# austin-hoover/ment-flow

Hardware: AMD Instinct MI355X
Metric: particle-samples/sec per MENT-Flow train step (6D, 100 proj) (higher is better)
Workload: dtype f32; 1 GPU; c4: rec_nd_1d gaussian_mixture d=6, 100 linear 1-D projections x 64 bins, NSF 5x[3x64] K=20; global_batch=2097152, per_gpu_batch=2097152, parallelism=dp1 (particle batch sharded; 2 all-reduces/step), step=zero_grad + MENTFlow.loss + backward + AdamW.step

## Files before the change

mentflow_amd/csrc/flow.hip:

```cpp
#include "flow_launch.h"
#include <stdlib.h>

namespace mf {

static int flow_check(int d, int L, int64_t n) {
    if (d < 1 || d > FLOW_DMAX) return fail("flow kernels support 1 <= d <= %d (got %d)", FLOW_DMAX, d);
    if (L < 1) return fail("hidden_layers must be >= 1");
    if (n < 0) return fail("negative particle count");
    return 0;
}

static int flow_grid(int64_t n, int waves = FLOW_WAVES) {
    const int64_t ntiles = (n + 31) / 32;
    int64_t g = (ntiles + waves - 1) / waves;
    if (g > NUM_CU) g = NUM_CU;
    if (g < 1) g = 1;
    return (int)g;
}

static int no_rqs_instance(int bins, int hidden_layers) {
    return fail("no RQS kernel instance for bins=%d hidden_layers=%d (built: 2 <= bins <= 21, hidden_layers in {1,2,3,4})", bins,
                hidden_layers);
}
static int no_affine_instance(int hidden_layers) {
    return fail("no affine kernel instance for hidden_layers=%d (built: 1 .. 4)", hidden_layers);
}

}

using namespace mf;

extern "C" int64_t mf_flow_image_floats(int d, int hidden_layers) { return image_layout(d, hidden_layers, d).total; }

static int g_bwd_variant = -1;
static bool bwd_fused_wanted() {
    static const int env_default = [] { const char* e = getenv("MENTFLOW_BWD_FUSED"); return (e && atoi(e) == 0) ? 0 : 1; }();
    return (g_bwd_variant < 0 ? env_default : g_bwd_variant) != 0;
}
extern "C" int mf_flow_set_bwd_variant(int variant) {
    if (variant < -1 || variant > 1) return fail("mf_flow_set_bwd_variant: -1 (default), 0 (two-kernel) or 1 (fused)");
    g_bwd_variant = variant;
    return 0;
}

static bool rqs_bwd_fused(int64_t n, int d, int hidden_layers, const int32_t* order, const Sparsity& sp, size_t* smem) {
    if (!bwd_fused_wanted() || order == nullptr || d > FB_DMAX) return false;
    (void)n;
    size_t fl = image_layout(d, hidden_layers, d).offW3;
    for (int i = 0; i < d; ++i) fl += (size_t)WS * (2 * ((sp.kend3[i] + 3) & ~3));
    fl += (size_t)d * HID + HID;
    fl = (fl + 3) & ~(size_t)3;
    *smem = sizeof(float) * (fl + 8 * (size_t)FB_TILE);
    return *smem <= 160 * 1024;
}

extern "C" int64_t mf_flow_bwd_scratch_floats(int64_t n, int d, int hidden_layers, const int32_t* order) {
    if (order != nullptr && d >= 1 && d <= FLOW_DMAX) {
        size_t smem;
        if (rqs_bwd_fused(n, d, hidden_layers, order, make_sparsity(d, order, d), &smem)) return 0;
    }
    const int64_t npad = ((n + 31) / 32) * 32;
    return (2 * (int64_t)hidden_layers + d) * npad * 64;
}

extern "C" int mf_flow_rqs_deriv_slot(int bins) {
    if (bins == 20 || bins == 8) return bins;
    return (bins >= 2 && bins <= RQS_KMAX) ? RQS_KMAX : -1;
}

extern "C" int mf_flow_rqs_act_level(int d, int hidden_layers, int bins, const int32_t* order) {
    if (order == nullptr || d < 1 || d > FLOW_DMAX || !rqs_saved_instance(bins, hidden_layers)) return 0;
    size_t smem;
    return rqs_bwd_fused(1, d, hidden_layers, order, make_sparsity(d, order, d), &smem) ? 2 : 0;
}
extern "C" int64_t mf_flow_rqs_act_floats(int64_t n, int d, int hidden_layers, int bins, int level) {
    if (n <= 0 || d < 1 || hidden_layers < 1 || level < 1 || level > 2) return 0;
    const int phif = bins == 20 ? phi_floats<20>() : (bins == 8 ? phi_floats<8>() : phi_floats<RQS_ANY>());
    return ((n + 31) / 32) * (int64_t)act_tile_floats(hidden_layers, level, d - 1, phif);
}

static int rqs_layer_fwd_impl(const float* image, int d, int hidden_layers, int bins, const int32_t* order, const float* x,
                              int64_t n, float* y, const float* logp_in, float* logp_out, int init_logp, float* act, int level,
                              void* stream);

extern "C" int mf_flow_rqs_layer_fwd(const float* image, int d, int hidden_layers, int bins, const int32_t* order,
                                      const float* x, int64_t n, float* y, const float* logp_in, float* logp_out,
                                      int init_logp, void* stream) {
    return rqs_layer_fwd_impl(image, d, hidden_layers, bins, order, x, n, y, logp_in, logp_out, init_logp, nullptr, 0, stream);
}

extern "C" int mf_flow_rqs_layer_fwd_save(const float* image, int d, int hidden_layers, int bins, const int32_t* order,
                                           const float* x, int64_t n, float* y, const float* logp_in, float* logp_out,
                                           int init_logp, float* act, int64_t act_floats, int level, void* stream) {
    if (level < 1 || level > 2) return fail("mf_flow_rqs_layer_fwd_save: level must be 1 or 2 (got %d)", level);
    if (level > mf_flow_rqs_act_level(d, hidden_layers, bins, order))
        return fail("no backward kernel consumes saved activations for d=%d hidden_layers=%d bins=%d (mf_flow_rqs_act_level)", d,
                    hidden_layers, bins);
    if (n > 0 && (act == nullptr || act_floats < mf_flow_rqs_act_floats(n, d, hidden_layers, bins, level)))
        return fail("act buffer too small: %lld floats, need %lld (mf_flow_rqs_act_floats)", (long long)act_floats,
                    (long long)mf_flow_rqs_act_floats(n, d, hidden_layers, bins, level));
    return rqs_layer_fwd_impl(image, d, hidden_layers, bins, order, x, n, y, logp_in, logp_out, init_logp, act, level, stream);
}

static int rqs_layer_fwd_impl(const float* image, int d, int hidden_layers, int bins, const int32_t* order, const float* x,
                              int64_t n, float* y, const float* logp_in, float* logp_out, int init_logp, float* act, int level,
                              void* stream) {
    if (flow_check(d, hidden_layers, n)) return 1;
    if (n == 0) return 0;
    const Sparsity sp = make_sparsity(d, order, d);
    const size_t smem = sizeof(float) * (size_t)image_layout(d, hidden_layers, d).total;
    const int64_t nt = (n + 31) / 32;
    const int fwd_block = nt <= 4 * NUM_CU ? 256 : (nt <= 8 * NUM_CU ? 512 : 1024);
    ProfScope prof(PK_FLOW_FWD, stream);
    if (launch_rqs_fwd(bins, hidden_layers, fwd_block, flow_grid(n, fwd_block / 64), smem, stream, image, d, x, n, y, logp_in,
                       logp_out, init_logp, sp, act, level))
        return no_rqs_instance(bins, hidden_layers);
    return check_launch("mf_flow_rqs_layer_fwd");
}

static int fused_grid(int64_t n) {
    const int64_t ngroups = ((n + 31) / 32 + 3) / 4;
    int64_t cap = NUM_CU;
#ifdef MF_EMU
    if (const char* e = getenv("MENTFLOW_EMU_FUSED_GRID")) cap = atoi(e) > 0 ? atoi(e) : cap;
#endif
    return (int)(ngroups > cap ? cap : (ngroups < 1 ? 1 : ngroups));
}
static int outer_accum_grid(int64_t n) {
    const int64_t ntiles = (n + 31) / 32;
    int64_t G = (ntiles + 7) / 8;
    if (G > 2 * NUM_CU) G = 2 * NUM_CU;
    if (G < 1) G = 1;
    return (int)G;
}

extern "C" int mf_flow_bwd_slab_rows(int64_t n, int d, int hidden_layers, const int32_t* order) {
    if (n <= 0) return 0;
    if (order != nullptr && d >= 1 && d <= FLOW_DMAX) {
        size_t smem;
        if (rqs_bwd_fused(n, d, hidden_layers, order, make_sparsity(d, order, d), &smem)) return fused_grid(n);
    }
    return outer_accum_grid(n);
}

extern "C" int mf_flow_rqs_layer_bwd_saved(const float* image, int d, int hidden_layers, int bins, const int32_t* order,
                                            const float* x, int64_t n, const float* gy, const float* glogp, float* gx,
                                            float* gslab, int slab_rows, int accumulate, const float* act, int64_t act_floats,
                                            int level, void* stream) {
    if (flow_check(d, hidden_layers, n)) return 1;
    if (n == 0) return 0;
    if (level < 1 || level > 2) return fail("mf_flow_rqs_layer_bwd_saved: level must be 1 or 2 (got %d)", level);
    if (level > mf_flow_rqs_act_level(d, hidden_layers, bins, order))
        return fail("no backward kernel consumes saved activations for d=%d hidden_layers=%d bins=%d (mf_flow_rqs_act_level)", d,
                    hidden_layers, bins);
    if (act == nullptr || act_floats < mf_flow_rqs_act_floats(n, d, hidden_layers, bins, level)) return fail("act buffer too small");
    const Sparsity sp = make_sparsity(d, order, d);
    size_t smem_f = 0;
    if (!rqs_bwd_fused(n, d, hidden_layers, order, sp, &smem_f)) return fail("the saved-activation backward is the fused kernel");
    if (slab_rows != fused_grid(n)) return fail("gslab has %d rows, this call writes %d (mf_flow_bwd_slab_rows)", slab_rows, fused_grid(n));
    ProfScope prof(PK_FLOW_BWD, stream);
    const int rc = level == 1 ? launch_rqs_bwd_fused_s1(bins, hidden_layers, fused_grid(n), smem_f, stream, image, d, x, n, gy, glogp,
                                                        gx, gslab, accumulate, sp, act)
                              : launch_rqs_bwd_fused_s2(bins, hidden_layers, fused_grid(n), smem_f, stream, image, d, x, n, gy, glogp,
// ... 173 lines not shown
```

mentflow_amd/csrc/flow_kernels.inc:

```
#include "common.h"
#include <stdlib.h>

namespace mf {

constexpr int HID = 64;
constexpr int WS = HID + 1;
constexpr int FLOW_BLOCK = 512;
constexpr int FLOW_WAVES = FLOW_BLOCK / WAVE;
constexpr int FLOW_DMAX = 7;
constexpr float RQS_BOUND = 5.0f;
constexpr float LOG_SLOPE_INV = 1.0f / 6.907755278982137f;

__device__ __forceinline__ constexpr int rowmap(int r, int hh) { return (r & 3) + 8 * (r >> 2) + 4 * hh; }

struct ImageLayout {
    int S0, offW0, offB0, offWh, offW3, offB3, total;
};
__host__ __device__ inline ImageLayout image_layout(int d, int L, int nblk) {
    ImageLayout g;
    g.S0 = d | 1;
    g.offW0 = 0;
    g.offB0 = HID * g.S0;
    g.offWh = g.offB0 + HID;
    g.offW3 = g.offWh + (L - 1) * (HID * WS + HID);
    g.offB3 = g.offW3 + nblk * HID * WS;
    g.total = g.offB3 + nblk * HID;
    return g;
}

typedef float f32x16_t __attribute__((ext_vector_type(16)));

struct Sparsity {
    int kend_h[2];
    int kbeg_ht[2];
    int kend3[FLOW_DMAX + 1];
    int rt1[FLOW_DMAX + 1];
};

static Sparsity make_sparsity(int d, const int32_t* order, int nblk) {
    Sparsity sp;
    sp.kend_h[0] = sp.kend_h[1] = 32;
    sp.kbeg_ht[0] = sp.kbeg_ht[1] = 0;
    for (int i = 0; i <= FLOW_DMAX; ++i) { sp.kend3[i] = 32; sp.rt1[i] = 1; }
    if (order == nullptr || d < 2) return sp;
    int cum[FLOW_DMAX + 2];
    for (int c = 0; c <= d; ++c) {
        int cnt = 0;
        for (int u = 0; u < HID; ++u) cnt += (1 + u % (d - 1)) <= c;
        cum[c] = cnt;
    }
    auto class_of = [&](int j) { int c = 1; while (cum[c] <= j) ++c; return c; };
    for (int rt = 0; rt < 2; ++rt) {
        sp.kend_h[rt] = (cum[class_of(32 * rt + 31)] + 1) / 2;
        sp.kbeg_ht[rt] = cum[class_of(32 * rt) - 1] / 2;
    }
    if (nblk == d) {
        for (int i = 0; i < d; ++i) {
            sp.kend3[i] = (cum[order[i]] + 1) / 2;
            sp.rt1[i] = cum[order[i]] > 32;
        }
    } else {
        sp.kend3[0] = 32;
        sp.rt1[0] = 1;
    }
    return sp;
}

#define MF_NO_HOIST() asm volatile("" ::: "memory")

__device__ __forceinline__ f32x16_t mfma(float a, float b, f32x16_t c) {
    return __builtin_amdgcn_mfma_f32_32x32x2f32(a, b, c, 0, 0, 0);
}

template <int BLOCK = FLOW_BLOCK>
__device__ __forceinline__ void stage_image(float* lds, const float* __restrict__ image, int total) {
    for (int i = threadIdx.x * 4; i < total; i += BLOCK * 4)
        *reinterpret_cast<float4*>(lds + i) = *reinterpret_cast<const float4*>(image + i);
    __syncthreads();
}

__device__ __forceinline__ f32x16_t bias_tile(const float* b, int rt, int hh) {
    f32x16_t acc;
#pragma unroll
    for (int r = 0; r < 16; ++r) acc[r] = b[32 * rt + rowmap(r, hh)];
    return acc;
}

__device__ __forceinline__ constexpr int kcol(int s) { return 32 * (s >> 4) + rowmap(s & 15, 0); }

__device__ __forceinline__ void linear64s(const float* W, int stride, const float* b, const f32x16_t (&in)[2],
                                          f32x16_t (&out)[2], int col, int hh, int kend0, int kend1) {
#pragma unroll
    for (int rt = 0; rt < 2; ++rt) {
        f32x16_t acc = bias_tile(b, rt, hh);
        const float* wrow = W + (32 * rt + col) * stride + 4 * hh;
        const int kend = rt ? kend1 : kend0;
#pragma unroll
        for (int s4 = 0; s4 < 32; s4 += 4) {
            if (s4 < kend) {
                float a[4];
#pragma unroll
                for (int j = 0; j < 4; ++j) a[j] = wrow[kcol(s4 + j)];
#pragma unroll
                for (int j = 0; j < 4; ++j) acc = mfma(a[j], in[(s4 + j) >> 4][(s4 + j) & 15], acc);
            }
        }
        out[rt] = acc;
    }
}
__device__ __forceinline__ void linear64(const float* W, const float* b, const f32x16_t (&in)[2], f32x16_t (&out)[2],
                                         int col, int hh, int kend0, int kend1) {
    linear64s(W, WS, b, in, out, col, hh, kend0, kend1);
}

__device__ __forceinline__ void linear64_t(const float* W, const f32x16_t (&in)[2], f32x16_t (&out)[2], int col, int hh,
                                           int kbeg0, int kbeg1) {
#pragma unroll
    for (int rt = 0; rt < 2; ++rt) {
        f32x16_t acc = out[rt];
        const float* wcol = W + 4 * hh * WS + 32 * rt + col;
        const int kbeg = rt ? kbeg1 : kbeg0;
#pragma unroll
        for (int s4 = 0; s4 < 32; s4 += 4) {
            if (s4 + 4 > kbeg) {
                float a[4];
#pragma unroll
                for (int j = 0; j < 4; ++j) a[j] = wcol[kcol(s4 + j) * WS];
#pragma unroll
                for (int j = 0; j < 4; ++j) acc = mfma(a[j], in[(s4 + j) >> 4][(s4 + j) & 15], acc);
            }
        }
// ... 77 lines not shown
__device__ __forceinline__ void half_pair(int v, int hh, int& lo, int& hi) {
#ifdef MF_EMU
    const int o = __shfl_xor(v, 32);
    lo = hh ? o : v;
    hi = hh ? v : o;
#else
    (void)hh;
    const auto r = __builtin_amdgcn_permlane32_swap((unsigned)v, (unsigned)v, false, false);
    lo = (int)r[0];
    hi = (int)r[1];
#endif
}

__device__ __forceinline__ unsigned cvt_u32_sat(float f) {
#ifdef MF_EMU
    return !(f > 0.0f) ? 0u : (f >= 4294967296.0f ? 0xffffffffu : (unsigned)f);
#else
    unsigned r;
    asm("v_cvt_u32_f32_e32 %0, %1" : "=v"(r) : "v"(f));
    return r;
#endif
}

template <int N, typename T>
__device__ __forceinline__ void select_pair(const T (&t)[N + 1], int idx, T& lo, T& hi) {
    constexpr int M = (N + 1) / 2;
    T a[M][3];
#pragma unroll
    for (int j = 0; j < M; ++j) {
        a[j][0] = t[2 * j];
        a[j][1] = t[2 * j + 1 <= N ? 2 * j + 1 : N];
        a[j][2] = t[2 * j + 2 <= N ? 2 * j + 2 : N];
    }
    const int j2 = idx >> 1;
#pragma unroll
    for (int b = 0; (1 << b) < M; ++b) {
        const bool bit = ((j2 >> b) & 1) != 0;
#pragma unroll
        for (int j = 0; j + (1 << b) < M; j += 2 << b)
#pragma unroll
            for (int c = 0; c < 3; ++c) a[j][c] = bit ? a[j + (1 << b)][c] : a[j][c];
    }
    const bool odd = (idx & 1) != 0;
    lo = odd ? a[0][1] : a[0][0];
    hi = odd ? a[0][2] : a[0][1];
}

constexpr int RQS_ANY = -1;
constexpr int RQS_KMAX = 21;
#define MF_PHASE(name) ((void)0)
struct NoSink {
    __device__ __forceinline__ void operator()(int, float) const {}
};
template <int K, int MODE, class Sink = NoSink>
__device__ __forceinline__ void rqs_apply(const float (&v)[32], float x, int hh, float& y_out, float& ladj_out,
                                          float gy, float gl, float (&g)[32], float& gx_out, int kbins = 0,
                                          const Sink& sink = Sink()) {
    constexpr int KM = K > 0 ? K : RQS_KMAX;
    constexpr int KD0M = KM / 2;
    const int kb = K > 0 ? K : kbins;
    const int KD0 = kb / 2;
    const int KD1 = kb - 1 - KD0;
    constexpr float A2 = 2.0f * LOG_SLOPE_INV;
    constexpr float A1 = LOG_SLOPE_INV;
    constexpr float FIX = 2147483648.0f;
    static_assert(KM + KD0M <= 32, "spline does not fit the 32 slots of a lane half");
#define MF_BIN_ON(m) (K > 0 || (m) < kb)

    MF_PHASE("softclip_exp");
    float p[KM], pq[MODE == 1 ? KM : 1];
    float sum = 0.0f;
#pragma unroll
    for (int m = 0; m < KM; ++m) {
        const float ia = fast_rcp(fmaf(fabsf(v[m]), A2 / LOG2E, 1.0f / LOG2E));
        p[m] = MF_BIN_ON(m) ? __builtin_amdgcn_exp2f(v[m] * ia) : 0.0f;
        if (MODE == 1) pq[m] = p[m] * (ia * ia);
        sum += p[m];
    }
    MF_PHASE("prefix_search");
    const float inv = fast_rcp(sum);
    unsigned cj[KM + 1];
    cj[0] = 0u;
    const float xc = fmaf(x, 0.5f / RQS_BOUND, 0.5f);
    const unsigned xq = cvt_u32_sat(xc * FIX);
    const float fscale = inv * FIX;
    unsigned c = 0u;
    int cnt = (-RQS_BOUND < x) ? 1 : 0;
#pragma unroll
    for (int j = 0; j < KM; ++j) {
        c += cvt_u32_sat(fmaf(p[j], fscale, 0.5f));
        cj[j + 1] = c;
        cnt += (MF_BIN_ON(j) && c < xq) ? 1 : 0;
    }
    MF_PHASE("select_knots");
    {
        int lo, hi;
        half_pair(cnt, hh, lo, hi);
        cnt = (MODE == 2) ? hi : lo;
    }
    const int k = cnt - 1;
    const bool inrange = (cnt >= 1) && (cnt <= kb);
    unsigned qk, qk1;
    select_pair<KM>(cj, min(max(k, 0), kb - 1), qk, qk1);
    const float ck = (float)qk * (1.0f / FIX), ck1 = (float)qk1 * (1.0f / FIX);
    const float kn0 = RQS_BOUND * (2.0f * ck - 1.0f);
    const float kn1 = RQS_BOUND * (2.0f * ck1 - 1.0f);
    float x0, x1, y0, y1;
    half_pair(kn0, hh, x0, y0);
    half_pair(kn1, hh, x1, y1);
    const int base = hh ? KD0 : 0;
    const int nown = hh ? KD1 : KD0;
    float r0, r1;
    {
        float G[KD0M + 4];
        G[0] = G[1] = G[KD0M + 2] = G[KD0M + 3] = 0.0f;
#pragma unroll
        for (int j = 0; j < KD0M; ++j) G[2 + j] = (j < nown) ? v[KM + j] : 0.0f;
        select_pair<KD0M + 3>(G, min(max(k - base + 1, 0), KD0M + 2), r0, r1);
    }
    {
        float a, b;
        half_pair(r0, hh, a, b);
        r0 = a + b;
        half_pair(r1, hh, a, b);
        r1 = a + b;
    }
    const float d0 = fast_exp(soft_clip(r0, A1));
    const float d1 = fast_exp(soft_clip(r1, A1));

    MF_PHASE("rational_log");
    const float w = x1 - x0;
    const float iw = fast_rcp(w);
    const float hgt = y1 - y0;
    const float s = hgt * iw;
    if (MODE == 2) {
        const float yb = x - y0;
        const float bet = d0 + d1 - 2.0f * s;
        const float qa = hgt * (s - d0) + yb * bet;
        const float qb = hgt * d0 - yb * bet;
        const float qc = -s * yb;
        const float zi = 2.0f * qc / (-qb - sqrtf(qb * qb - 4.0f * qa * qc));
        y_out = inrange ? fmaf(zi, w, x0) : x;
        ladj_out = 0.0f;
        return;
    }
    const float z = (x - x0) * iw;
    const float omz = 1.0f - z;
    const float z1 = z * omz;
    const float beta = d0 + d1 - 2.0f * s;
    const float num = s * z * z + d0 * z1;
    const float den = fmaf(beta, z1, s);
    const float iden = fast_rcp(den);
    const float R = num * iden;
    const float Q = 2.0f * s * z1 + d0 * omz * omz + d1 * z * z;
    const float jac = s * s * Q * iden * iden;
    y_out = inrange ? fmaf(hgt, R, y0) : x;
    ladj_out = inrange ? __builtin_amdgcn_logf(jac) * 0.6931471805599453f : 0.0f;

    MF_PHASE("adjoint_scalar");
    if (MODE == 1) {
        const float tz = 1.0f - 2.0f * z;
        const float num_z = 2.0f * s * z + d0 * tz;
        const float den_z = beta * tz;
        const float R_z = (num_z - R * den_z) * iden;
        const float den_s = 1.0f - 2.0f * z1;
        const float R_s = (z * z - R * den_s) * iden;
        const float R_d0 = z1 * (1.0f - R) * iden;
        const float R_d1 = -R * z1 * iden;
        const float iQ = fast_rcp(Q);
        const float Q_z = 2.0f * s * tz - 2.0f * d0 * omz + 2.0f * d1 * z;
        const float l_z = Q_z * iQ - 2.0f * den_z * iden;
        const float l_s = 2.0f * fast_rcp(s) + 2.0f * z1 * iQ - 2.0f * den_s * iden;
        const float l_d0 = omz * omz * iQ - 2.0f * z1 * iden;
        const float l_d1 = z * z * iQ - 2.0f * z1 * iden;
        const float gyh = gy * hgt;
        const float Gz = gyh * R_z + gl * l_z;
        const float Gs = gyh * R_s + gl * l_s;
        const float Gd0 = gyh * R_d0 + gl * l_d0;
        const float Gd1 = gyh * R_d1 + gl * l_d1;
        const float Gh = gy * R;
        gx_out = inrange ? Gz * iw : gy;
        const float gx0 = (Gz * (z - 1.0f) + Gs * s) * iw;
        const float gx1 = -(Gz * z + Gs * s) * iw;
        const float gy0 = gy - Gh - Gs * iw;
        const float gy1 = Gh + Gs * iw;
        const float gcA = inrange ? 2.0f * RQS_BOUND * (hh ? gy0 : gx0) : 0.0f;
        const float gcB = inrange ? 2.0f * RQS_BOUND * (hh ? gy1 : gx1) : 0.0f;
        const float dot = gcA * ck + gcB * ck1;
        MF_PHASE("adjoint_logits");
        const float nrm = inv * (1.0f / (LOG2E * LOG2E));
        const float t_gt = (0.0f - dot) * nrm, d_eq = gcB * nrm, d_lt = gcA * nrm;
        const float kf = (float)k;
        float u_prev = __builtin_amdgcn_fmed3f(kf + 1.0f, 0.0f, 1.0f);
#pragma unroll
        for (int m = 0; m < KM; ++m) {
            const float u = __builtin_amdgcn_fmed3f(kf - (float)m, 0.0f, 1.0f);
            g[m] = pq[m] * fmaf(u, d_lt, fmaf(u_prev, d_eq, t_gt));
            sink(m, g[m]);
            u_prev = u;
        }
        MF_PHASE("adjoint_derivs");
        const float gr0 = inrange ? Gd0 * d0 * soft_clip_grad(r0, A1) : 0.0f;
        const float gr1 = inrange ? Gd1 * d1 * soft_clip_grad(r1, A1) : 0.0f;
#pragma unroll
        for (int j = 0; j < 32 - KM; ++j) {
            const bool own = j < nown;
            float t = 0.0f;
            t = (own && (k - 1 == base + j)) ? gr0 : t;
            t = (own && (k == base + j)) ? t + gr1 : t;
            g[KM + j] = t;
            sink(KM + j, t);
        }
    }
    MF_PHASE("end");
}
#undef MF_BIN_ON

__device__ __forceinline__ void block_linear(const float* W, const float* b, const f32x16_t (&in)[2], float (&v)[32],
                                             int col, int hh, int kend) {
    f32x16_t phi[2];
    linear64(W, b, in, phi, col, hh, kend, kend);
#pragma unroll
    for (int m = 0; m < 32; ++m) v[m] = phi[m >> 4][m & 15];
}

__device__ __forceinline__ float base_log_prob(const float* xp, int d) {
    float q = 0.0f;
    for (int j = 0; j < d; ++j) q = fmaf(xp[j], xp[j], q);
    return -0.5f * q - 0.9189385332046727f * (float)d;
}

constexpr int ACT_BLOCK = 2048;
template <int K>
__host__ __device__ constexpr int phi_slots() { return K > 0 ? ((K + K / 2 + 1) & ~1) : 32; }
template <int K>
__host__ __device__ constexpr int phi_floats() { return 64 * phi_slots<K>(); }
__host__ __device__ inline int act_tile_floats(int L, int level, int nphi, int phif) {
    return level <= 0 ? 0 : (L - 1) * ACT_BLOCK + (level >= 2 ? nphi * phif : 0);
}

typedef float act_f4 __attribute__((ext_vector_type(4)));
typedef float act_f2 __attribute__((ext_vector_type(2)));
#ifdef MF_EMU
#define MF_ACT_ST(p, v) (*(p) = (v))
#define MF_ACT_LD(p) (*(p))
#else
#define MF_ACT_ST(p, v) __builtin_nontemporal_store((v), (p))
#define MF_ACT_LD(p) __builtin_nontemporal_load(p)
#endif
__device__ __forceinline__ void act_store(float* __restrict__ blk, int lane, const f32x16_t (&a)[2]) {
    act_f4* q = reinterpret_cast<act_f4*>(blk) + lane;
#pragma unroll
    for (int rt = 0; rt < 2; ++rt)
#pragma unroll
        for (int g4 = 0; g4 < 4; ++g4) {
            const act_f4 t = {a[rt][4 * g4], a[rt][4 * g4 + 1], a[rt][4 * g4 + 2], a[rt][4 * g4 + 3]};
            MF_ACT_ST(q + (4 * rt + g4) * 64, t);
        }
}
__device__ __forceinline__ void act_load(const float* __restrict__ blk, int lane, f32x16_t (&a)[2]) {
    const act_f4* q = reinterpret_cast<const act_f4*>(blk) + lane;
#pragma unroll
    for (int rt = 0; rt < 2; ++rt)
#pragma unroll
        for (int g4 = 0; g4 < 4; ++g4) {
            const act_f4 t = MF_ACT_LD(q + (4 * rt + g4) * 64);
            a[rt][4 * g4] = t.x;
            a[rt][4 * g4 + 1] = t.y;
            a[rt][4 * g4 + 2] = t.z;
            a[rt][4 * g4 + 3] = t.w;
        }
}
template <int K>
__device__ __forceinline__ void phi_store(float* __restrict__ blk, int lane, const float (&v)[32]) {
    constexpr int NS = phi_slots<K>(), NQ = NS / 4;
    act_f4* q = reinterpret_cast<act_f4*>(blk) + lane;
#pragma unroll
    for (int g4 = 0; g4 < NQ; ++g4) {
        const act_f4 t = {v[4 * g4], v[4 * g4 + 1], v[4 * g4 + 2], v[4 * g4 + 3]};
        MF_ACT_ST(q + g4 * 64, t);
    }
    if constexpr (NS % 4 != 0) {
        const act_f2 t = {v[4 * NQ], v[4 * NQ + 1]};
        MF_ACT_ST(reinterpret_cast<act_f2*>(blk + 256 * NQ) + lane, t);
    }
}
template <int K>
__device__ __forceinline__ void phi_load(const float* __restrict__ blk, int lane, float (&v)[32]) {
    constexpr int NS = phi_slots<K>(), NQ = NS / 4;
    const act_f4* q = reinterpret_cast<const act_f4*>(blk) + lane;
#pragma unroll
    for (int g4 = 0; g4 < NQ; ++g4) {
        const act_f4 t = MF_ACT_LD(q + g4 * 64);
        v[4 * g4] = t.x;
        v[4 * g4 + 1] = t.y;
        v[4 * g4 + 2] = t.z;
        v[4 * g4 + 3] = t.w;
    }
    if constexpr (NS % 4 != 0) {
        const act_f2 t = MF_ACT_LD(reinterpret_cast<const act_f2*>(blk + 256 * NQ) + lane);
        v[4 * NQ] = t.x;
        v[4 * NQ + 1] = t.y;
    }
#pragma unroll
    for (int m = NS; m < 32; ++m) v[m] = 0.0f;
}

template <int K, int L, int BLOCK>
__global__ __launch_bounds__(BLOCK) void rqs_layer_fwd_kernel(const float* __restrict__ image, int d,
                                                                   const float* __restrict__ x, int64_t n,
                                                                   float* __restrict__ y,
                                                                   const float* __restrict__ logp_in,
                                                                   float* __restrict__ logp_out, int init_logp,
                                                                   Sparsity sp, int bins_rt, float* __restrict__ act,
                                                                   int act_level) {
    MF_DYN_SMEM(float, lds);
    const ImageLayout g = image_layout(d, L, d);
    stage_image<BLOCK>(lds, image, g.total);
    const int lane = threadIdx.x & 63, wid = threadIdx.x >> 6, col = lane & 31, hh = lane >> 5;
    const int64_t ntiles = (n + 31) / 32;
    int nphi = 0;
    for (int i = 0; i < d; ++i) nphi += sp.kend3[i] > 0;
    const int act_tf = act_tile_floats(L, act_level, nphi, phi_floats<K>());
    for (int64_t tile = (int64_t)blockIdx.x * (BLOCK / 64) + wid; tile < ntiles; tile += (int64_t)gridDim.x * (BLOCK / 64)) {
        MF_NO_HOIST();
        const int64_t p = tile * 32 + col;
        const bool valid = p < n;
        const float* xp = x + (valid ? p : n - 1) * d;
        float* const ablk = act + tile * act_tf;
        float xb[4];
#pragma unroll
        for (int s = 0; s < 4; ++s) xb[s] = (2 * s + hh < d) ? xp[2 * s + hh] : 0.0f;
        int d_s = d, kh0 = sp.kend_h[0], kh1 = sp.kend_h[1];
#ifndef MF_EMU
        asm volatile("" : "+s"(d_s), "+s"(kh0), "+s"(kh1));
#endif
        f32x16_t h[2];
        input_layer(lds + g.offW0, lds + g.offB0, g.S0, d_s, xb, h, col, hh);
#pragma unroll
        for (int l = 1; l < L; ++l) {
            f32x16_t t[2];
            const float* W = lds + g.offWh + (l - 1) * (HID * WS + HID);
            linear64(W, W + HID * WS, h, t, col, hh, kh0, kh1);
            relu2(t);
            h[0] = t[0];
            h[1] = t[1];
            if (act_level >= 1) act_store(ablk + (l - 1) * ACT_BLOCK, lane, h);
        }
        float ladj = 0.0f;
        float* pphi = ablk + (L - 1) * ACT_BLOCK;
#pragma unroll 1
        for (int i = 0; i < d; ++i) {
            float v[32], gdummy[32];
            block_linear(lds + g.offW3 + i * HID * WS, lds + g.offB3 + i * HID, h, v, col, hh, sp.kend3[i]);
            if (act_level >= 2 && sp.kend3[i] > 0) {
                phi_store<K>(pphi, lane, v);
                pphi += phi_floats<K>();
            }
            float yi, li, gxd;
            rqs_apply<K, 0>(v, xp[i], hh, yi, li, 0.0f, 0.0f, gdummy, gxd, bins_rt);
            ladj += li;
            if (valid && hh == 0) y[p * d + i] = yi;
        }
        if (valid && hh == 0) {
            const float lp0 = init_logp ? base_log_prob(xp, d) : logp_in[p];
            logp_out[p] = lp0 - ladj;
        }
    }
}

__device__ __forceinline__ void store_tile(float* __restrict__ dst, int64_t tile, int col, int hh, const float (&v)[32]) {
    float* base = dst + tile * 2048 + (16 * hh) * 32 + col;
#pragma unroll
    for (int m = 0; m < 32; ++m) base[(32 * (m >> 4) + (m & 15)) * 32] = v[m];
}
__device__ __forceinline__ void store_tile(float* __restrict__ dst, int64_t tile, int col, int hh, const f32x16_t (&a)[2]) {
    float* base = dst + tile * 2048 + (16 * hh) * 32 + col;
#pragma unroll
    for (int rt = 0; rt < 2; ++rt)
#pragma unroll
        for (int r = 0; r < 16; ++r) base[(32 * rt + r) * 32] = a[rt][r];
}

template <int K, int L, int BLOCK>
__global__ __launch_bounds__(BLOCK) void rqs_layer_bwd_kernel(const float* __restrict__ image, int d,
                                                                   const float* __restrict__ x, int64_t n,
                                                                   const float* __restrict__ gy,
                                                                   const float* __restrict__ glogp,
                                                                   float* __restrict__ gx, float* __restrict__ scratch,
                                                                   Sparsity sp, int bins_rt) {
    MF_DYN_SMEM(float, lds);
    const ImageLayout g = image_layout(d, L, d);
    stage_image<BLOCK>(lds, image, g.total);
    const int lane = threadIdx.x & 63, wid = threadIdx.x >> 6, col = lane & 31, hh = lane >> 5;
    const int64_t ntiles = (n + 31) / 32;
    const int64_t npad = ntiles * 32;
    float* ACT = scratch;
    float* GPRE = ACT + (int64_t)L * npad * 64;
    float* GPHI = GPRE + (int64_t)L * npad * 64;
    for (int64_t tile = (int64_t)blockIdx.x * (BLOCK / 64) + wid; tile < ntiles; tile += (int64_t)gridDim.x * (BLOCK / 64)) {
        MF_NO_HOIST();
        const int64_t p = tile * 32 + col;
        const bool valid = p < n;
        const int64_t pc = valid ? p : n - 1;
        const float* xp = x + pc * d;
        float xb[4];
#pragma unroll
        for (int s = 0; s < 4; ++s) xb[s] = (2 * s + hh < d) ? xp[2 * s + hh] : 0.0f;
        f32x16_t h[L][2];
        input_layer(lds + g.offW0, lds + g.offB0, g.S0, d, xb, h[0], col, hh);
        store_tile(ACT, tile, col, hh, h[0]);
#pragma unroll
        for (int l = 1; l < L; ++l) {
// ... 519 lines not shown
__device__ __forceinline__ void pair_reduce_bias(float* X, int wid, int lane, float& bsum) {
    __syncthreads();
    if (wid & 1) X[(wid >> 1) * 64 + lane] = bsum;
    __syncthreads();
    if (!(wid & 1)) bsum += X[(wid >> 1) * 64 + lane];
}

#ifdef MF_FB_NO_BARRIER
#define FB_SYNC() ((void)0)
#else
#define FB_SYNC() __syncthreads()
#endif
#ifdef MF_FB_NO_DW
#define FB_DW(...) ((void)0)
#else
#define FB_DW(...) dw_accum(__VA_ARGS__)
#endif
#ifdef MF_FB_NO_SPLINE
#define FB_SPLINE(...)                                                                                               \
    do {                                                                                                             \
        _Pragma("unroll") for (int m_ = 0; m_ < 32; ++m_) gv[m_] = v[m_] * gyi;                                       \
        gxd = gl; yi = xi; li = 0.0f;                                                                                \
    } while (0)
#else
#define FB_SPLINE(...) __VA_ARGS__
#endif

template <int K, int L, int SAVED = 0>
__global__ __launch_bounds__(FB_BLOCK) void rqs_layer_bwd_fused_kernel(const float* __restrict__ image, int d,
                                                                        const float* __restrict__ x, int64_t n,
                                                                        const float* __restrict__ gy,
                                                                        const float* __restrict__ glogp,
                                                                        float* __restrict__ gx, float* __restrict__ gslab,
                                                                        int accumulate, Sparsity sp, int bins_rt,
                                                                        const float* __restrict__ act) {
    MF_DYN_SMEM(float, lds);
    const ImageLayout g = image_layout(d, L, d);
    float* gimage = gslab + (int64_t)blockIdx.x * g.total;
    for (int i = threadIdx.x * 4; i < g.offW3; i += FB_BLOCK * 4)
        *reinterpret_cast<float4*>(lds + i) = *reinterpret_cast<const float4*>(image + i);
    int off = g.offW3;
    for (int i = 0; i < d; ++i) {
        const int nc = fb_blk_cols(sp, i);
        for (int e = threadIdx.x; e < HID * nc; e += FB_BLOCK) {
            const int r = e / nc, c = e - r * nc;
            lds[off + c * WS + r] = image[g.offW3 + (i * HID + r) * WS + c];
        }
        off += nc * WS;
    }
    const int offB3c = off;
    for (int e = threadIdx.x; e < d * HID; e += FB_BLOCK) lds[offB3c + e] = image[g.offB3 + e];
    float* zrow = lds + offB3c + d * HID;
    if (threadIdx.x < HID) zrow[threadIdx.x] = 0.0f;
    float* SA = lds + ((offB3c + d * HID + HID + 3) & ~3);
    float* SB = SA + 4 * FB_TILE;
    __syncthreads();

    const int lane = threadIdx.x & 63, wid = __builtin_amdgcn_readfirstlane((int)(threadIdx.x >> 6)), col = lane & 31, hh = lane >> 5;
    float* myA = SA + wid * FB_TILE;
    float* myB = SB + wid * FB_TILE;
    const int fra = wid >> 1, frb = wid & 1;
    const int hra = wid & 1, ht0 = 2 * (wid >> 1);
#ifdef MF_ASM_CHAIN
    const DwRole role{fra, frb, hra, ht0};
#endif

    f32x16_t accO[FB_DMAX], accT[L];
    float bsO[FB_DMAX], bsT[L];
#pragma unroll
    for (int i = 0; i < FB_DMAX; ++i) {
        bsO[i] = 0.0f;
#pragma unroll
        for (int r = 0; r < 16; ++r) accO[i][r] = 0.0f;
    }
#pragma unroll
    for (int l = 0; l < L; ++l) {
        bsT[l] = 0.0f;
#pragma unroll
        for (int r = 0; r < 16; ++r) accT[l][r] = 0.0f;
    }

    unsigned long long c_[16] = {0, 0, 0, 0, 0, 0, 0, 0, 0, 0, 0, 0, 0, 0, 0, 0}, t0_, tl_, t1_;
    const int64_t ntiles = (n + 31) / 32;
    const int64_t ngroups = (ntiles + 3) / 4;
    float xn[FB_DMAX], gyn[FB_DMAX], gln;
    auto load_rows = [&](int64_t grp2, float (&xo)[FB_DMAX], float (&go)[FB_DMAX], float& glo) {
        const int64_t p2 = (grp2 * 4 + wid) * 32 + col;
        const bool v2 = p2 < n;
        const int64_t pc2 = v2 ? p2 : n - 1;
#pragma unroll
        for (int j = 0; j < FB_DMAX; ++j) {
            const int jc = j < d ? j : d - 1;
            const float xv = x[pc2 * d + jc], gv_ = gy[pc2 * d + jc];
            xo[j] = (j < d) ? xv : 0.0f;
            go[j] = (v2 && j < d) ? gv_ : 0.0f;
        }
        const float glv = glogp[pc2];
        glo = v2 ? -glv : 0.0f;
    };
    load_rows(blockIdx.x, xn, gyn, gln);
    int nphi = 0, ipure = -1;
    for (int i = 0; i < d; ++i) {
        nphi += sp.kend3[i] > 0;
        ipure = sp.kend3[i] > 0 ? ipure : i;
    }
    const int act_tf = act_tile_floats(L, SAVED, nphi, phi_floats<K>());
    auto act_tile = [&](int64_t grp2) {
// ... 45 lines not shown
            f32x16_t h0[2];
            input_layer4(lds + g.offW0, lds + g.offB0, g.S0, xb, h0, col, hh);
#pragma unroll
            for (int l = 1; l < L; ++l) {
                const float* W = lds + g.offWh + (l - 1) * (HID * WS + HID);
                h[l][0] = bias_tile(W + HID * WS, 0, hh);
                h[l][1] = bias_tile(W + HID * WS, 1, hh);
                {
                    const float* w0 = W + col * WS + 4 * hh;
                    const float* w1 = W + (32 + col) * WS + 4 * hh;
                    const BTile bt{l == 1 ? h0 : h[l - 1]};
                    switch ((sp.kend_h[0] + 3) >> 2) {
                        case 4: chain64x2r<1, 0, 4, 0, 8>(h[l][0], h[l][1], w0, w1, bt); break;
                        case 5: chain64x2r<1, 0, 5, 0, 8>(h[l][0], h[l][1], w0, w1, bt); break;
                        case 6: chain64x2r<1, 0, 6, 0, 8>(h[l][0], h[l][1], w0, w1, bt); break;
                        default: chain64x2i<1, 8>(h[l][0], h[l][1], w0, w1, bt); break;
                    }
                }
                if (l == L - 1) {
                    FB_SYNC();
                    relu2_stage(h[l], myB, lane);
                } else {
                    relu2(h[l]);
                }
            }
            if (L == 1) { h[0][0] = h0[0]; h[0][1] = h0[1]; }
        }
        WS_ACC(c_[0], t0_);
        if (L == 1 && SAVED == 0) {
            FB_SYNC();
            stage_tile(myB, lane, h[L - 1]);
        }
        f32x16_t gh[2];
        f32x16_t gacc;
#pragma unroll
        for (int r = 0; r < 16; ++r) {
            gh[0][r] = 0.0f;
            gh[1][r] = 0.0f;
            gacc[r] = 0.0f;
        }
        int w3off = g.offW3;
        auto feature = [&](int i, f32x16_t& accF, float& bsF) {
            float v[32], gv[32];
            int kend3_i = sp.kend3[0], rt1_i = sp.rt1[0];
#pragma unroll
            for (int j = 1; j < FB_DMAX; ++j) {
                kend3_i = (i == j) ? sp.kend3[j] : kend3_i;
                rt1_i = (i == j) ? sp.rt1[j] : rt1_i;
            }
            const int nc = 2 * ((kend3_i + 3) & ~3);
            const float* W3 = lds + w3off;
            w3off += nc * WS;
            t0_ = WS_T();
            if constexpr (SAVED >= 2) {
                if (kend3_i > 0) {
#pragma unroll
                    for (int m = 0; m < 32; ++m) v[m] = vn[m];
                } else {
#pragma unroll
                    for (int m = 0; m < 32; ++m) v[m] = lds[offB3c + i * HID + 32 * (m >> 4) + rowmap(m & 15, hh)];
                }
            } else {
                f32x16_t phi[2];
                phi[0] = bias_tile(lds + offB3c + i * HID, 0, hh);
                phi[1] = bias_tile(lds + offB3c + i * HID, 1, hh);
                chain64x2_upto<WS>(phi[0], phi[1], W3 + 4 * hh * WS + col, W3 + 4 * hh * WS + 32 + col, (kend3_i + 3) >> 2,
                                   BTile{h[L - 1]});
#pragma unroll
                for (int m = 0; m < 32; ++m) v[m] = phi[m >> 4][m & 15];
            }
            WS_ACC(c_[1], t0_);
            t0_ = WS_T();
            float xi = xr[0], gyi = gyr[0];
#pragma unroll
            for (int j = 1; j < FB_DMAX; ++j) {
                xi = (i == j) ? xr[j] : xi;
                gyi = (i == j) ? gyr[j] : gyi;
            }
            float yi, li, gxd;
            if (i > 0) FB_SYNC();
#if defined(MF_FB_NO_SPLINE)
            FB_SPLINE(rqs_apply<K, 1>(v, xi, hh, yi, li, gyi, gl, gv, gxd, bins_rt));
            stage_tile(myA, lane, gv);
#else
            {
                float* const qA = myA + lane;
                auto to_stage = [qA](int m, float val) { qA[m * FB_PS] = val; };
                rqs_apply<K, 1>(v, xi, hh, yi, li, gyi, gl, gv, gxd, bins_rt, to_stage);
            }
#endif
            WS_ACC(c_[2], t0_);
            if constexpr (SAVED >= 2) {
                if (kend3_i > 0 && nphi > 0) {
                    const int nx = next_saved(i);
                    phi_load<K>(nx < d ? phi_blk(ablk, nx) : phi_blk(act_tile(grp_next), first_saved), lane, vn);
                }
            }
#pragma unroll
            for (int j = 0; j < 4; ++j) gacc[j] += ((hh == ((i >> 2) & 1)) && ((i & 3) == j)) ? gxd : 0.0f;
            t0_ = WS_T();
            WS_ACC(c_[4], t0_);
            t0_ = WS_T();
            if (kend3_i > 0) {
                const float* r0 = (col < nc ? W3 + col * WS : zrow) + 4 * hh;
                if (rt1_i != 0) {
                    const float* r1 = (32 + col < nc ? W3 + (32 + col) * WS : zrow) + 4 * hh;
                    if constexpr (K == 20) chain64x2i<1, 8, true>(gh[0], gh[1], r0, r1, BVec{gv});
                    else chain64x2i<1, 8>(gh[0], gh[1], r0, r1, BVec{gv});
                } else {
                    if constexpr (K == 20) chain64_30<1>(gh[0], r0, BVec{gv});
                    else chain64<1>(gh[0], r0, 0, 8, BVec{gv});
                }
            }
            WS_ACC(c_[8], t0_);
            t0_ = WS_T();
            FB_SYNC();
            WS_ACC(c_[5], t0_);
            t0_ = WS_T();
            {
                const bool full = rt1_i != 0;
                const bool mm = kend3_i > 0;
#if defined(MF_ASM_CHAIN) && !defined(MF_FB_NO_DW)
                dw_product_stage(SA, SB, role, full, mm, lane, accF, bsF);
#else
                FB_DW(SA, SB, full ? fra : hra, full ? frb : 0, full ? 0 : ht0, full ? 2 : 1, mm, full ? frb : -1, lane, accF, bsF);
#endif
                WS_ACC(c_[6], t0_);
            }
        };
        static_assert(FB_DMAX % 2 == 0, "two features per iteration");
#pragma unroll 1
        for (int i = 0; i < FB_DMAX; i += 2) {
            if (i < d) feature(i, accO[0], bsO[0]);
            if (i + 1 < d) feature(i + 1, accO[1], bsO[1]);
            const f32x16_t ta0 = accO[0], ta1 = accO[1];
            const float tb0 = bsO[0], tb1 = bsO[1];
#pragma unroll
            for (int k = 0; k + 2 < FB_DMAX; ++k) {
                accO[k] = accO[k + 2];
                bsO[k] = bsO[k + 2];
            }
            accO[FB_DMAX - 2] = ta0;
            accO[FB_DMAX - 1] = ta1;
            bsO[FB_DMAX - 2] = tb0;
// ... 678 lines not shown
```

Baseline: 99.74 million particle-samples/s.

## Precompute spline parameters for the input-independent first coupling feature into an LDS table

For the feature whose conditioner has no inputs (kend3 == 0), the spline parameters (softclip exponentials, normalized cumulative knots, derivative logits) depend only on the bias. They are now built once per block by wave 0 into a small LDS table and loaded per tile, so that feature skips the per-particle exp/rcp/prefix work in both the forward and the fused backward kernels. rqs_apply is split into rqs_params, rqs_search and rqs_eval to support this. The change adds LDS usage and an extra sync after the table build, and it only helps the one pure feature out of d.

```diff
diff --git a/mentflow_amd/csrc/flow.hip b/mentflow_amd/csrc/flow.hip
--- a/mentflow_amd/csrc/flow.hip
+++ b/mentflow_amd/csrc/flow.hip
@@ -49,7 +49,7 @@
     size_t fl = image_layout(d, hidden_layers, d).offW3;
     for (int i = 0; i < d; ++i) fl += (size_t)WS * (2 * ((sp.kend3[i] + 3) & ~3));
     fl += (size_t)d * HID + HID;
-    fl = (fl + 3) & ~(size_t)3;
+    fl = ((fl + 3) & ~(size_t)3) + RQS_TAB_FLOATS;
     *smem = sizeof(float) * (fl + 8 * (size_t)FB_TILE);
     return *smem <= 160 * 1024;
 }
@@ -108,7 +108,7 @@
     if (flow_check(d, hidden_layers, n)) return 1;
     if (n == 0) return 0;
     const Sparsity sp = make_sparsity(d, order, d);
-    const size_t smem = sizeof(float) * (size_t)image_layout(d, hidden_layers, d).total;
+    const size_t smem = sizeof(float) * (size_t)(fwd_table_offset(image_layout(d, hidden_layers, d).total) + RQS_TAB_FLOATS);
     const int64_t nt = (n + 31) / 32;
     const int fwd_block = nt <= 4 * NUM_CU ? 256 : (nt <= 8 * NUM_CU ? 512 : 1024);
     ProfScope prof(PK_FLOW_FWD, stream);
diff --git a/mentflow_amd/csrc/flow_kernels.inc b/mentflow_amd/csrc/flow_kernels.inc
--- a/mentflow_amd/csrc/flow_kernels.inc
+++ b/mentflow_amd/csrc/flow_kernels.inc
@@ -72,11 +72,11 @@
     return __builtin_amdgcn_mfma_f32_32x32x2f32(a, b, c, 0, 0, 0);
 }
 
-template <int BLOCK = FLOW_BLOCK>
+template <int BLOCK = FLOW_BLOCK, bool SYNC = true>
 __device__ __forceinline__ void stage_image(float* lds, const float* __restrict__ image, int total) {
     for (int i = threadIdx.x * 4; i < total; i += BLOCK * 4)
         *reinterpret_cast<float4*>(lds + i) = *reinterpret_cast<const float4*>(image + i);
-    __syncthreads();
+    if (SYNC) __syncthreads();
 }
 
 __device__ __forceinline__ f32x16_t bias_tile(const float* b, int rt, int hh) {
@@ -260,46 +260,152 @@
 struct NoSink {
     __device__ __forceinline__ void operator()(int, float) const {}
 };
+template <int K, int MODE>
+struct RqsParams {
+    static constexpr int KM = K > 0 ? K : RQS_KMAX;
+    static constexpr int KD0M = KM / 2;
+    unsigned cj[KM + 1];
+    float pq[MODE == 1 ? KM : 1];
+    float inv;
+    float dl[KD0M];
+};
+#define MF_BIN_ON(m) (K > 0 || (m) < kb)
+template <int K, int MODE, bool SEARCH = true>
+__device__ __forceinline__ void rqs_params(const float (&v)[32], RqsParams<K, MODE>& P, float x, int& cnt, int kbins = 0) {
+    constexpr int KM = RqsParams<K, MODE>::KM, KD0M = RqsParams<K, MODE>::KD0M;
+    const int kb = K > 0 ? K : kbins;
+    constexpr float A2 = 2.0f * LOG_SLOPE_INV;
+    constexpr float FIX = 2147483648.0f;
+    static_assert(KM + KD0M <= 32, "spline does not fit the 32 slots of a lane half");
+    MF_PHASE("softclip_exp");
+    float p[KM];
+    float sum = 0.0f;
+#pragma unroll
+    for (int m = 0; m < KM; ++m) {
+        const float ia = fast_rcp(fmaf(fabsf(v[m]), A2 / LOG2E, 1.0f / LOG2E));
+        p[m] = MF_BIN_ON(m) ? __builtin_amdgcn_exp2f(v[m] * ia) : 0.0f;
+        if (MODE == 1) P.pq[m] = p[m] * (ia * ia);
+        sum += p[m];
+    }
+    MF_PHASE("prefix_search");
+    P.inv = fast_rcp(sum);
+    P.cj[0] = 0u;
+    const float xc = fmaf(x, 0.5f / RQS_BOUND, 0.5f);
+    const unsigned xq = cvt_u32_sat(xc * FIX);
+    const float fscale = P.inv * FIX;
+    unsigned c = 0u;
+    cnt = (-RQS_BOUND < x) ? 1 : 0;
+#pragma unroll
+    for (int j = 0; j < KM; ++j) {
+        c += cvt_u32_sat(fmaf(p[j], fscale, 0.5f));
+        P.cj[j + 1] = c;
+        if (SEARCH) cnt += (MF_BIN_ON(j) && c < xq) ? 1 : 0;
+    }
+#pragma unroll
+    for (int j = 0; j < KD0M; ++j) P.dl[j] = v[KM + j];
+    MF_PHASE("end");
+}
+template <int K, int MODE>
+__device__ __forceinline__ int rqs_search(const RqsParams<K, MODE>& P, float x, int kbins = 0) {
+    constexpr int KM = RqsParams<K, MODE>::KM;
+    const int kb = K > 0 ? K : kbins;
+    constexpr float FIX = 2147483648.0f;
+    MF_PHASE("order0_search");
+    const float xc = fmaf(x, 0.5f / RQS_BOUND, 0.5f);
+    const unsigned xq = cvt_u32_sat(xc * FIX);
+    int cnt = (-RQS_BOUND < x) ? 1 : 0;
+#pragma unroll
+    for (int j = 0; j < KM; ++j) cnt += (MF_BIN_ON(j) && P.cj[j + 1] < xq) ? 1 : 0;
+    MF_PHASE("end");
+    return cnt;
+}
+
+constexpr int RQS_TAB_HALF = 64;
+constexpr int RQS_TAB_FLOATS = 2 * RQS_TAB_HALF;
+__host__ __device__ inline int fwd_table_offset(int image_total) { return (image_total + 3) & ~3; }
+template <int K>
+struct RqsTable {
+    static constexpr int KM = K > 0 ? K : RQS_KMAX, KD0M = KM / 2;
+    static constexpr int NCJ4 = (KM + 2 + 3) / 4;
+    static constexpr int NPQ4 = (KM + 3) / 4;
+    static constexpr int NDL4 = (KD0M + 3) / 4;
+    static constexpr int PQ = 4 * NCJ4, DL = PQ + 4 * NPQ4;
+    static_assert(DL + 4 * NDL4 <= RQS_TAB_HALF, "table does not fit");
+};
+typedef unsigned tab_u4 __attribute__((ext_vector_type(4)));
+template <int K, int MODE>
+__device__ __forceinline__ void rqs_table_build(float* tab, const float* __restrict__ b, int lane, int kbins) {
+    typedef RqsTable<K> T;
+    const int col = lane & 31, hh = lane >> 5;
+    float v[32];
+#pragma unroll
+    for (int m = 0; m < 32; ++m) v[m] = b[32 * (m >> 4) + rowmap(m & 15, hh)];
+    RqsParams<K, MODE> P;
+    int cnt;
+    rqs_params<K, MODE, false>(v, P, 0.0f, cnt, kbins);
+    if (col == 0) {
+        float* t = tab + hh * RQS_TAB_HALF;
+#pragma unroll
+        for (int j = 0; j <= T::KM; ++j) t[j] = __builtin_bit_cast(float, P.cj[j]);
+        t[T::KM + 1] = P.inv;
+        if (MODE == 1) {
+#pragma unroll
+            for (int j = 0; j < T::KM; ++j) t[T::PQ + j] = P.pq[j];
+        }
+#pragma unroll
+        for (int j = 0; j < T::KD0M; ++j) t[T::DL + j] = P.dl[j];
+    }
+}
+template <int K, int MODE>
+__device__ __forceinline__ void rqs_table_load(const float* tab, int hh, RqsParams<K, MODE>& P) {
+    typedef RqsTable<K> T;
+    MF_PHASE("order0_table_load");
+    const tab_u4* t = reinterpret_cast<const tab_u4*>(tab + hh * RQS_TAB_HALF);
+    unsigned w[4 * T::NCJ4], q[4 * T::NPQ4], e[4 * T::NDL4];
+#pragma unroll
+    for (int j = 0; j < T::NCJ4; ++j) {
+        const tab_u4 u = t[j];
+        w[4 * j] = u.x; w[4 * j + 1] = u.y; w[4 * j + 2] = u.z; w[4 * j + 3] = u.w;
+    }
+    if (MODE == 1) {
+#pragma unroll
+        for (int j = 0; j < T::NPQ4; ++j) {
+            const tab_u4 u = t[T::NCJ4 + j];
+            q[4 * j] = u.x; q[4 * j + 1] = u.y; q[4 * j + 2] = u.z; q[4 * j + 3] = u.w;
+        }
+    }
+#pragma unroll
+    for (int j = 0; j < T::NDL4; ++j) {
+        const tab_u4 u = t[T::NCJ4 + T::NPQ4 + j];
+        e[4 * j] = u.x; e[4 * j + 1] = u.y; e[4 * j + 2] = u.z; e[4 * j + 3] = u.w;
+    }
+#pragma unroll
+    for (int j = 0; j <= T::KM; ++j) P.cj[j] = w[j];
+    P.inv = __builtin_bit_cast(float, w[T::KM + 1]);
+    if (MODE == 1) {
+#pragma unroll
+        for (int j = 0; j < T::KM; ++j) P.pq[j] = __builtin_bit_cast(float, q[j]);
+    }
+#pragma unroll
+    for (int j = 0; j < T::KD0M; ++j) P.dl[j] = __builtin_bit_cast(float, e[j]);
+    MF_PHASE("end");
+}
+
 template <int K, int MODE, class Sink = NoSink>
-__device__ __forceinline__ void rqs_apply(const float (&v)[32], float x, int hh, float& y_out, float& ladj_out,
-                                          float gy, float gl, float (&g)[32], float& gx_out, int kbins = 0,
-                                          const Sink& sink = Sink()) {
-    constexpr int KM = K > 0 ? K : RQS_KMAX;
-    constexpr int KD0M = KM / 2;
+__device__ __forceinline__ void rqs_eval(const RqsParams<K, MODE>& P, int cnt, float x, int hh, float& y_out,
+                                         float& ladj_out, float gy, float gl, float (&g)[32], float& gx_out, int kbins = 0,
+                                         const Sink& sink = Sink()) {
+    constexpr int KM = RqsParams<K, MODE>::KM, KD0M = RqsParams<K, MODE>::KD0M;
     const int kb = K > 0 ? K : kbins;
     const int KD0 = kb / 2;
     const int KD1 = kb - 1 - KD0;
-    constexpr float A2 = 2.0f * LOG_SLOPE_INV;
     constexpr float A1 = LOG_SLOPE_INV;
     constexpr float FIX = 2147483648.0f;
-    static_assert(KM + KD0M <= 32, "spline does not fit the 32 slots of a lane half");
-#define MF_BIN_ON(m) (K > 0 || (m) < kb)
-
-    MF_PHASE("softclip_exp");
-    float p[KM], pq[MODE == 1 ? KM : 1];
-    float sum = 0.0f;
-#pragma unroll
-    for (int m = 0; m < KM; ++m) {
-        const float ia = fast_rcp(fmaf(fabsf(v[m]), A2 / LOG2E, 1.0f / LOG2E));
-        p[m] = MF_BIN_ON(m) ? __builtin_amdgcn_exp2f(v[m] * ia) : 0.0f;
-        if (MODE == 1) pq[m] = p[m] * (ia * ia);
-        sum += p[m];
-    }
-    MF_PHASE("prefix_search");
-    const float inv = fast_rcp(sum);
-    unsigned cj[KM + 1];
-    cj[0] = 0u;
-    const float xc = fmaf(x, 0.5f / RQS_BOUND, 0.5f);
-    const unsigned xq = cvt_u32_sat(xc * FIX);
-    const float fscale = inv * FIX;
-    unsigned c = 0u;
-    int cnt = (-RQS_BOUND < x) ? 1 : 0;
-#pragma unroll
-    for (int j = 0; j < KM; ++j) {
-        c += cvt_u32_sat(fmaf(p[j], fscale, 0.5f));
-        cj[j + 1] = c;
-        cnt += (MF_BIN_ON(j) && c < xq) ? 1 : 0;
-    }
+    const unsigned (&cj)[KM + 1] = P.cj;
+    const float (&pq)[MODE == 1 ? KM : 1] = P.pq;
+    const float inv = P.inv;
+    (void)pq;
+    (void)inv;
     MF_PHASE("select_knots");
     {
         int lo, hi;
@@ -323,7 +429,7 @@
         float G[KD0M + 4];
         G[0] = G[1] = G[KD0M + 2] = G[KD0M + 3] = 0.0f;
 #pragma unroll
-        for (int j = 0; j < KD0M; ++j) G[2 + j] = (j < nown) ? v[KM + j] : 0.0f;
+        for (int j = 0; j < KD0M; ++j) G[2 + j] = (j < nown) ? P.dl[j] : 0.0f;
         select_pair<KD0M + 3>(G, min(max(k - base + 1, 0), KD0M + 2), r0, r1);
     }
     {
@@ -423,6 +529,15 @@
     MF_PHASE("end");
 }
 #undef MF_BIN_ON
+template <int K, int MODE, class Sink = NoSink>
+__device__ __forceinline__ void rqs_apply(const float (&v)[32], float x, int hh, float& y_out, float& ladj_out,
+                                          float gy, float gl, float (&g)[32], float& gx_out, int kbins = 0,
+                                          const Sink& sink = Sink()) {
+    RqsParams<K, MODE> P;
+    int cnt;
+    rqs_params<K, MODE>(v, P, x, cnt, kbins);
+    rqs_eval<K, MODE>(P, cnt, x, hh, y_out, ladj_out, gy, gl, g, gx_out, kbins, sink);
+}
 
 __device__ __forceinline__ void block_linear(const float* W, const float* b, const f32x16_t (&in)[2], float (&v)[32],
                                              int col, int hh, int kend) {
@@ -524,11 +639,17 @@
                                                                    int act_level) {
     MF_DYN_SMEM(float, lds);
     const ImageLayout g = image_layout(d, L, d);
-    stage_image<BLOCK>(lds, image, g.total);
+    stage_image<BLOCK, false>(lds, image, g.total);
     const int lane = threadIdx.x & 63, wid = threadIdx.x >> 6, col = lane & 31, hh = lane >> 5;
     const int64_t ntiles = (n + 31) / 32;
-    int nphi = 0;
-    for (int i = 0; i < d; ++i) nphi += sp.kend3[i] > 0;
+    int nphi = 0, ipure = -1;
+    for (int i = 0; i < d; ++i) {
+        nphi += sp.kend3[i] > 0;
+        ipure = sp.kend3[i] > 0 ? ipure : i;
+    }
+    float* const tab = lds + fwd_table_offset(g.total);
+    if (wid == 0 && ipure >= 0) rqs_table_build<K, 0>(tab, image + g.offB3 + ipure * HID, lane, bins_rt);
+    __syncthreads();
     const int act_tf = act_tile_floats(L, act_level, nphi, phi_floats<K>());
     for (int64_t tile = (int64_t)blockIdx.x * (BLOCK / 64) + wid; tile < ntiles; tile += (int64_t)gridDim.x * (BLOCK / 64)) {
         MF_NO_HOIST();
@@ -559,14 +680,24 @@
         float* pphi = ablk + (L - 1) * ACT_BLOCK;
 #pragma unroll 1
         for (int i = 0; i < d; ++i) {
-            float v[32], gdummy[32];
-            block_linear(lds + g.offW3 + i * HID * WS, lds + g.offB3 + i * HID, h, v, col, hh, sp.kend3[i]);
-            if (act_level >= 2 && sp.kend3[i] > 0) {
-                phi_store<K>(pphi, lane, v);
-                pphi += phi_floats<K>();
+            float gdummy[32];
+            RqsParams<K, 0> P;
+            int cnt;
+            const float xi = xp[i];
+            if (sp.kend3[i] > 0) {
+                float v[32];
+                block_linear(lds + g.offW3 + i * HID * WS, lds + g.offB3 + i * HID, h, v, col, hh, sp.kend3[i]);
+                if (act_level >= 2) {
+                    phi_store<K>(pphi, lane, v);
+                    pphi += phi_floats<K>();
+                }
+                rqs_params<K, 0>(v, P, xi, cnt, bins_rt);
+            } else {
+                rqs_table_load<K, 0>(tab, hh, P);
+                cnt = rqs_search<K, 0>(P, xi, bins_rt);
             }
             float yi, li, gxd;
-            rqs_apply<K, 0>(v, xp[i], hh, yi, li, 0.0f, 0.0f, gdummy, gxd, bins_rt);
+            rqs_eval<K, 0>(P, cnt, xi, hh, yi, li, 0.0f, 0.0f, gdummy, gxd, bins_rt);
             ladj += li;
             if (valid && hh == 0) y[p * d + i] = yi;
         }
@@ -1192,7 +1323,13 @@
     for (int e = threadIdx.x; e < d * HID; e += FB_BLOCK) lds[offB3c + e] = image[g.offB3 + e];
     float* zrow = lds + offB3c + d * HID;
     if (threadIdx.x < HID) zrow[threadIdx.x] = 0.0f;
-    float* SA = lds + ((offB3c + d * HID + HID + 3) & ~3);
+    float* const tab = lds + ((offB3c + d * HID + HID + 3) & ~3);
+    {
+        int ip = -1;
+        for (int i = 0; i < d; ++i) ip = sp.kend3[i] > 0 ? ip : i;
+        if ((threadIdx.x >> 6) == 0 && ip >= 0) rqs_table_build<K, 1>(tab, image + g.offB3 + ip * HID, threadIdx.x & 63, bins_rt);
+    }
+    float* SA = tab + RQS_TAB_FLOATS;
     float* SB = SA + 4 * FB_TILE;
     __syncthreads();
 
@@ -1344,6 +1481,11 @@
             const float* W3 = lds + w3off;
             w3off += nc * WS;
             t0_ = WS_T();
+#if !defined(MF_FB_NO_SPLINE)
+            RqsParams<K, 1> P;
+            if (kend3_i == 0) rqs_table_load<K, 1>(tab, hh, P);
+            else
+#endif
             if constexpr (SAVED >= 2) {
                 if (kend3_i > 0) {
 #pragma unroll
@@ -1376,12 +1518,16 @@
             stage_tile(myA, lane, gv);
 #else
             {
+                int cnt;
+                if (kend3_i > 0) rqs_params<K, 1>(v, P, xi, cnt, bins_rt);
+                else cnt = rqs_search<K, 1>(P, xi, bins_rt);
                 float* const qA = myA + lane;
                 auto to_stage = [qA](int m, float val) { qA[m * FB_PS] = val; };
-                rqs_apply<K, 1>(v, xi, hh, yi, li, gyi, gl, gv, gxd, bins_rt, to_stage);
+                rqs_eval<K, 1>(P, cnt, xi, hh, yi, li, gyi, gl, gv, gxd, bins_rt, to_stage);
             }
 #endif
             WS_ACC(c_[2], t0_);
+            if (kend3_i == 0) WS_ACC(c_[3], t0_);
             if constexpr (SAVED >= 2) {
                 if (kend3_i > 0 && nphi > 0) {
                     const int nx = next_saved(i);
```

Measured after the change: 100.5 million particle-samples/s, median of 6. Within noise of the previous version (+0.8%).
